# zhuangshaobin/Video-GPT

Hardware: AMD Instinct MI355X
Metric: denoised clip-tokens/sec (256^2, 8-frame next-clip, CFG, x1) (higher is better)
Workload: dtype bf16; 1 GPU; cfg-2 single-GPU inference: 256^2, C=4 cond + G=8 gen frames, CFG (B=2, L=3096, 5160 real tokens), Phi-3-mini-class denoiser 32 layers, x1 prediction, hipGraph sampler step; global_batch=1, parallelism=replicas x1, graph=True, condition_prefix_reuse=True, special_row_hoisting=True, attention_precision=bf16, full=False

## Files before the change

video-gpt_amd/csrc/glue.hip:

```cpp
#include "common.h"

namespace {

__global__ __launch_bounds__(256) void embed_gather_kernel(const int64_t* __restrict__ ids,
                                                           const bf16* __restrict__ table,
                                                           bf16* __restrict__ out, int64_t rows,
                                                           int H, int64_t vocab) {
    const int cpr = H >> 3;
    const int64_t total = rows * cpr;
    for (int64_t i = (int64_t)blockIdx.x * blockDim.x + threadIdx.x; i < total;
         i += (int64_t)gridDim.x * blockDim.x) {
        const int64_t row = i / cpr;
        const int c = (int)(i % cpr);
        int64_t id = ids[row];
        id = id < 0 ? 0 : (id >= vocab ? vocab - 1 : id);
        *reinterpret_cast<bf16x8*>(out + row * H + c * 8) =
            *reinterpret_cast<const bf16x8*>(table + id * H + c * 8);
    }
}

__global__ __launch_bounds__(256) void patch_embed_kernel(
    const bf16* __restrict__ x, const bf16* __restrict__ Wp, const bf16* __restrict__ bias,
    const bf16* __restrict__ pos, const int32_t* __restrict__ dst_row, bf16* __restrict__ seq,
    int C, int h, int w, int H, int pos_max) {
    __shared__ float patch[16][16];
    const int f = blockIdx.y;
    const int h2 = h >> 1, w2 = w >> 1;
    const int ntok = h2 * w2;
    const int t0 = blockIdx.x * 16;
    {
        const int tl = threadIdx.x >> 4, e = threadIdx.x & 15;
        const int t = t0 + tl;
        float v = 0.f;
        if (t < ntok) {
            const int ci = e >> 2, p = (e >> 1) & 1, q = e & 1;
            const int i = t / w2, j = t % w2;
            v = bf2f(x[(((int64_t)f * C + ci) * h + 2 * i + p) * w + 2 * j + q]);
        }
        patch[tl][e] = v;
    }
    __syncthreads();
    const int top = (pos_max - h2) / 2, left = (pos_max - w2) / 2;
    const int64_t row0 = dst_row[f];
    for (int c0 = threadIdx.x * 4; c0 < H; c0 += 256 * 4) {
        float wreg[4][16];
#pragma unroll
        for (int cc = 0; cc < 4; ++cc) {
            const bf16x8 lo = *reinterpret_cast<const bf16x8*>(Wp + (int64_t)(c0 + cc) * 16);
            const bf16x8 hi = *reinterpret_cast<const bf16x8*>(Wp + (int64_t)(c0 + cc) * 16 + 8);
#pragma unroll
            for (int e = 0; e < 8; ++e) {
                wreg[cc][e] = bf2f(lo[e]);
                wreg[cc][8 + e] = bf2f(hi[e]);
            }
        }
        const bf16x4 bv = *reinterpret_cast<const bf16x4*>(bias + c0);
        for (int tl = 0; tl < 16; ++tl) {
            const int t = t0 + tl;
            if (t >= ntok) break;
            const int i = t / w2, j = t % w2;
            const bf16x4 pv = *reinterpret_cast<const bf16x4*>(
                pos + ((int64_t)(top + i) * pos_max + left + j) * H + c0);
            bf16x4 o;
#pragma unroll
            for (int cc = 0; cc < 4; ++cc) {
                float acc = 0.f;
#pragma unroll
                for (int e = 0; e < 16; ++e) acc += wreg[cc][e] * patch[tl][e];
                o[cc] = f2bf(acc + bf2f(bv[cc]) + bf2f(pv[cc]));
            }
            *reinterpret_cast<bf16x4*>(seq + (row0 + t) * H + c0) = o;
        }
    }
}

__global__ void timestep_sinusoid_kernel(const float* __restrict__ t, const float* __restrict__ freqs,
                                         bf16* __restrict__ out, int n, int half) {
    const int idx = blockIdx.x * blockDim.x + threadIdx.x;
    if (idx >= n * half) return;
    const int m = idx / half, i = idx % half;
    const float arg = t[m] * freqs[i];
    out[(int64_t)m * 2 * half + i] = f2bf(cosf(arg));
    out[(int64_t)m * 2 * half + half + i] = f2bf(sinf(arg));
}

template <int MT>
__global__ __launch_bounds__(256) void linear_small_kernel(
    const bf16* __restrict__ x, const bf16* __restrict__ W, const bf16* __restrict__ bias,
    bf16* __restrict__ out, const int32_t* __restrict__ out_row, int M, int N, int K, int64_t ldx,
    int64_t ldo, int pre_act, int post_act) {
    const int lane = threadIdx.x & 63;
    const int wave = threadIdx.x >> 6;
    for (int n = blockIdx.x * 4 + wave; n < N; n += gridDim.x * 4) {
        float acc[MT];
#pragma unroll
        for (int m = 0; m < MT; ++m) acc[m] = 0.f;
        const bf16* wr = W + (int64_t)n * K;
        for (int k = lane * 8; k < K; k += 512) {
            const bf16x8 wv = *reinterpret_cast<const bf16x8*>(wr + k);
            float wf[8];
#pragma unroll
            for (int j = 0; j < 8; ++j) wf[j] = bf2f(wv[j]);
#pragma unroll
            for (int m = 0; m < MT; ++m) {
                if (m < M) {
                    const bf16x8 xv = *reinterpret_cast<const bf16x8*>(x + (int64_t)m * ldx + k);
#pragma unroll
                    for (int j = 0; j < 8; ++j) {
                        float xf = bf2f(xv[j]);
                        if (pre_act != VGPT_ACT_NONE) xf = bf2f(f2bf(act_apply(xf, pre_act)));
                        acc[m] += wf[j] * xf;
                    }
                }
            }
        }
        const float bn = bias ? bf2f(bias[n]) : 0.f;
#pragma unroll
        for (int m = 0; m < MT; ++m) {
            if (m < M) {
                float v = wave_sum(acc[m]) + bn;
                v = act_apply(v, post_act);
                if (lane == 0) {
                    const int64_t r = out_row ? (int64_t)out_row[m] : (int64_t)m;
                    out[r * ldo + n] = f2bf(v);
                }
            }
        }
    }
}

template <int NCH>
__global__ __launch_bounds__(256) void final_layer_kernel(
    const bf16* __restrict__ hidden, const int32_t* __restrict__ src_row, const bf16* __restrict__ mod,
    const bf16* __restrict__ Wf, const bf16* __restrict__ bfin, bf16* __restrict__ out, int C, int h,
    int w, int H, float eps) {
    const int lane = threadIdx.x & 63;
    const int wave = threadIdx.x >> 6;
    const int f = blockIdx.y;
    const int h2 = h >> 1, w2 = w >> 1;
    const int ntok = h2 * w2;
    const int t = blockIdx.x * 4 + wave;
    if (t >= ntok) return;
    const bf16* xr = hidden + ((int64_t)src_row[f] + t) * H;
    const bf16* shift = mod + (int64_t)f * 2 * H;
    const bf16* scale = shift + H;
    float v[NCH][8];
    float s1 = 0.f;
#pragma unroll
    for (int c = 0; c < NCH; ++c) {
        const int off = (c * 64 + lane) * 8;
        if (off < H) {
            const bf16x8 xv = *reinterpret_cast<const bf16x8*>(xr + off);
#pragma unroll
            for (int j = 0; j < 8; ++j) {
                v[c][j] = bf2f(xv[j]);
                s1 += v[c][j];
            }
        } else {
#pragma unroll
            for (int j = 0; j < 8; ++j) v[c][j] = 0.f;
        }
    }
    const float mean = wave_sum(s1) / (float)H;
    float s2 = 0.f;
#pragma unroll
    for (int c = 0; c < NCH; ++c) {
        const int off = (c * 64 + lane) * 8;
        if (off < H) {
#pragma unroll
            for (int j = 0; j < 8; ++j) {
                const float d = v[c][j] - mean;
                s2 += d * d;
            }
        }
    }
    const float rstd = rsqrtf(wave_sum(s2) / (float)H + eps);
#pragma unroll
    for (int c = 0; c < NCH; ++c) {
        const int off = (c * 64 + lane) * 8;
        if (off < H) {
            const bf16x8 sh = *reinterpret_cast<const bf16x8*>(shift + off);
            const bf16x8 sc = *reinterpret_cast<const bf16x8*>(scale + off);
#pragma unroll
            for (int j = 0; j < 8; ++j)
                v[c][j] = (v[c][j] - mean) * rstd * (1.0f + bf2f(sc[j])) + bf2f(sh[j]);
        }
    }
    float y = 0.f;
    for (int o = 0; o < 16; ++o) {
        float acc = 0.f;
#pragma unroll
        for (int c = 0; c < NCH; ++c) {
            const int off = (c * 64 + lane) * 8;
            if (off < H) {
                const bf16x8 wv = *reinterpret_cast<const bf16x8*>(Wf + (int64_t)o * H + off);
#pragma unroll
                for (int j = 0; j < 8; ++j) acc += v[c][j] * bf2f(wv[j]);
            }
        }
        acc = wave_sum(acc);
        if (lane == o) y = acc + bf2f(bfin[o]);
    }
    if (lane < 16) {
        const int c = lane % C, pq = lane / C;
        const int p = pq >> 1, q = pq & 1;
        const int i = t / w2, j = t % w2;
        out[(((int64_t)f * C + c) * h + 2 * i + p) * w + 2 * j + q] = f2bf(y);
    }
}

__global__ void set_timesteps_kernel(const float* sigma, const int32_t* step, float* ts, int n, int n_steps) {
    const int i = blockIdx.x * blockDim.x + threadIdx.x;
    const int st = *step;
    if (i < n && st >= 0 && st <= n_steps) ts[i] = sigma[st];
}

__global__ __launch_bounds__(256) void euler_cfg_kernel(float* __restrict__ z, bf16* __restrict__ zm,
                                                        const bf16* __restrict__ pred,
                                                        const float* __restrict__ sigma,
                                                        const int32_t* __restrict__ step, int n_steps, int n_frames,
                                                        int64_t elems, int pred_type, int use_cfg,
                                                        float cfg_scale) {
    const int st = *step;
    if (st < 0 || st >= n_steps) return;
    const float sg = sigma[st], sg_next = sigma[st + 1];
    const float dt = sg_next - sg;
    const float inv = 1.0f / (1.0f - sg);
    const int half = use_cfg ? n_frames / 2 : n_frames;
    const int64_t total = (int64_t)half * elems;
    for (int64_t i = (int64_t)blockIdx.x * blockDim.x + threadIdx.x; i < total;
         i += (int64_t)gridDim.x * blockDim.x) {
        float zc = z[i];
        float vc = bf2f(pred[i]);
        if (pred_type == VGPT_PRED_X1) vc = (vc - zc) * inv;
        if (use_cfg) {
            const int64_t iu = i + total;
            float zu = z[iu];
            float vu = bf2f(pred[iu]);
            if (pred_type == VGPT_PRED_X1) vu = (vu - zu) * inv;
            vc = vu + cfg_scale * (vc - vu);
            zu += dt * vc;
            z[iu] = zu;
            zm[iu] = f2bf(zu);
        }
        zc += dt * vc;
        z[i] = zc;
        zm[i] = f2bf(zc);
    }
}

__global__ void advance_kernel(int32_t* step) { *step += 1; }

__global__ __launch_bounds__(256) void cast_f32_bf16_kernel(const float* __restrict__ src,
                                                            bf16* __restrict__ dst, int64_t n) {
    for (int64_t i = (int64_t)blockIdx.x * blockDim.x + threadIdx.x; i < n;
         i += (int64_t)gridDim.x * blockDim.x)
        dst[i] = f2bf(src[i]);
}

}

VGPT_EXPORT int vgpt_embed_gather(const int64_t* ids, const void* table, void* out, int64_t rows,
                                  int64_t H, int64_t vocab, void* stream) {
    VGPT_REQUIRE(ids && table && out, VGPT_ERR_INVALID, "vgpt_embed_gather: null pointer");
    VGPT_REQUIRE(rows >= 0 && H > 0 && vocab > 0, VGPT_ERR_INVALID, "vgpt_embed_gather: bad shape");
    VGPT_REQUIRE(H % 8 == 0, VGPT_ERR_UNSUPPORTED, "vgpt_embed_gather: H must be a multiple of 8");
    if (rows == 0) return VGPT_OK;
    int grid = (int)std::min<int64_t>(cdiv(rows * (H / 8), 256), (int64_t)1 << 30);
    hipLaunchKernelGGL(embed_gather_kernel, dim3(grid), dim3(256), 0, (hipStream_t)stream, ids,
                       (const bf16*)table, (bf16*)out, rows, (int)H, vocab);
    VGPT_CHECK_LAUNCH("vgpt_embed_gather");
    return VGPT_OK;
}

VGPT_EXPORT int vgpt_patch_embed_fwd(const void* x, const void* Wp, const void* bias,
                                     const void* pos_embed, const int32_t* dst_row, void* seq,
                                     int n_frames, int C, int h, int w, int64_t H, int pos_max,
                                     void* stream) {
    VGPT_REQUIRE(x && Wp && bias && pos_embed && dst_row && seq, VGPT_ERR_INVALID,
                 "vgpt_patch_embed_fwd: null pointer");
    VGPT_REQUIRE(n_frames >= 0 && C > 0 && h > 0 && w > 0 && H > 0, VGPT_ERR_INVALID,
                 "vgpt_patch_embed_fwd: bad shape");
    VGPT_REQUIRE(C * 4 == 16 && h % 2 == 0 && w % 2 == 0, VGPT_ERR_UNSUPPORTED,
                 "vgpt_patch_embed_fwd: needs in_channels=4, patch 2, even latent size");
    VGPT_REQUIRE(H % 4 == 0, VGPT_ERR_UNSUPPORTED, "vgpt_patch_embed_fwd: H must be a multiple of 4");
    VGPT_REQUIRE(h / 2 <= pos_max && w / 2 <= pos_max, VGPT_ERR_INVALID,
                 "vgpt_patch_embed_fwd: latent larger than pos_embed_max_size");
    if (n_frames == 0) return VGPT_OK;
    const int ntok = (h / 2) * (w / 2);
    hipLaunchKernelGGL(patch_embed_kernel, dim3((unsigned)cdiv(ntok, 16), n_frames), dim3(256), 0,
                       (hipStream_t)stream, (const bf16*)x, (const bf16*)Wp, (const bf16*)bias,
                       (const bf16*)pos_embed, dst_row, (bf16*)seq, C, h, w, (int)H, pos_max);
    VGPT_CHECK_LAUNCH("vgpt_patch_embed_fwd");
    return VGPT_OK;
}

VGPT_EXPORT int vgpt_timestep_sinusoid(const float* t, const float* freqs, void* out, int n,
                                       int half, void* stream) {
    VGPT_REQUIRE(t && freqs && out, VGPT_ERR_INVALID, "vgpt_timestep_sinusoid: null pointer");
    VGPT_REQUIRE(n >= 0 && half > 0, VGPT_ERR_INVALID, "vgpt_timestep_sinusoid: bad shape");
    if (n == 0) return VGPT_OK;
    hipLaunchKernelGGL(timestep_sinusoid_kernel, dim3((unsigned)cdiv((int64_t)n * half, 256)),
                       dim3(256), 0, (hipStream_t)stream, t, freqs, (bf16*)out, n, half);
    VGPT_CHECK_LAUNCH("vgpt_timestep_sinusoid");
    return VGPT_OK;
}

VGPT_EXPORT int vgpt_linear_small(const void* x, const void* W, const void* bias, void* out,
                                  const int32_t* out_row, int M, int64_t N, int64_t K, int64_t ldx,
                                  int64_t ldo, int pre_act, int post_act, void* stream) {
    VGPT_REQUIRE(x && W && out, VGPT_ERR_INVALID, "vgpt_linear_small: null pointer");
    VGPT_REQUIRE(M >= 0 && N > 0 && K > 0, VGPT_ERR_INVALID, "vgpt_linear_small: bad shape");
    VGPT_REQUIRE(M <= 32, VGPT_ERR_UNSUPPORTED, "vgpt_linear_small: M=%d > 32", M);
    VGPT_REQUIRE(K % 8 == 0 && ldx % 8 == 0, VGPT_ERR_UNSUPPORTED,
                 "vgpt_linear_small: K and ldx must be multiples of 8");
    VGPT_REQUIRE(N < (1ll << 31) && K < (1ll << 31), VGPT_ERR_UNSUPPORTED,
                 "vgpt_linear_small: dimension too large");
    if (M == 0) return VGPT_OK;
    int grid = (int)std::min<int64_t>(cdiv(N, 4), 256 * 8);
    hipStream_t s = (hipStream_t)stream;
#define LS_CASE(MT)                                                                               \
    hipLaunchKernelGGL(linear_small_kernel<MT>, dim3(grid), dim3(256), 0, s, (const bf16*)x,       \
                       (const bf16*)W, (const bf16*)bias, (bf16*)out, out_row, M, (int)N, (int)K, \
                       ldx, ldo, pre_act, post_act)
    if (M <= 8) LS_CASE(8);
    else if (M <= 16) LS_CASE(16);
    else LS_CASE(32);
#undef LS_CASE
    VGPT_CHECK_LAUNCH("vgpt_linear_small");
    return VGPT_OK;
}

VGPT_EXPORT int vgpt_final_layer_fwd(const void* hidden, const int32_t* src_row, const void* mod,
                                     const void* Wf, const void* bf, void* out, int n_frames, int C,
                                     int h, int w, int64_t H, float eps, void* stream) {
    VGPT_REQUIRE(hidden && src_row && mod && Wf && bf && out, VGPT_ERR_INVALID,
                 "vgpt_final_layer_fwd: null pointer");
    VGPT_REQUIRE(n_frames >= 0 && C > 0 && h > 0 && w > 0 && H > 0, VGPT_ERR_INVALID,
                 "vgpt_final_layer_fwd: bad shape");
    VGPT_REQUIRE(C * 4 == 16 && h % 2 == 0 && w % 2 == 0, VGPT_ERR_UNSUPPORTED,
                 "vgpt_final_layer_fwd: needs out_channels=4, patch 2, even latent size");
    VGPT_REQUIRE(H % 8 == 0 && H <= 8 * 512, VGPT_ERR_UNSUPPORTED,
                 "vgpt_final_layer_fwd: H must be a multiple of 8 and <= 4096");
    if (n_frames == 0) return VGPT_OK;
    const int ntok = (h / 2) * (w / 2);
    dim3 grid((unsigned)cdiv(ntok, 4), n_frames);
    hipStream_t s = (hipStream_t)stream;
#define FL_CASE(N)                                                                              \
    case N:                                                                                     \
        hipLaunchKernelGGL(final_layer_kernel<N>, grid, dim3(256), 0, s, (const bf16*)hidden,   \
                           src_row, (const bf16*)mod, (const bf16*)Wf, (const bf16*)bf,         \
                           (bf16*)out, C, h, w, (int)H, eps);                                   \
        break;
    switch ((int)cdiv(H, 512)) {
        FL_CASE(1) FL_CASE(2) FL_CASE(3) FL_CASE(4) FL_CASE(5) FL_CASE(6) FL_CASE(7) FL_CASE(8)
    }
#undef FL_CASE
    VGPT_CHECK_LAUNCH("vgpt_final_layer_fwd");
    return VGPT_OK;
}

VGPT_EXPORT int vgpt_sampler_set_timesteps(const float* sigma, const int32_t* step, int n_steps, float* timesteps,
                                           int n, void* stream) {
    VGPT_REQUIRE(sigma && step && timesteps, VGPT_ERR_INVALID,
                 "vgpt_sampler_set_timesteps: null pointer");
    VGPT_REQUIRE(n >= 0 && n_steps > 0, VGPT_ERR_INVALID, "vgpt_sampler_set_timesteps: bad shape");
    if (n == 0) return VGPT_OK;
    hipLaunchKernelGGL(set_timesteps_kernel, dim3((unsigned)cdiv(n, 64)), dim3(64), 0,
                       (hipStream_t)stream, sigma, step, timesteps, n, n_steps);
    VGPT_CHECK_LAUNCH("vgpt_sampler_set_timesteps");
    return VGPT_OK;
}

VGPT_EXPORT int vgpt_euler_cfg_update(float* z, void* z_model, const void* pred, const float* sigma,
                                      const int32_t* step, int n_steps, int n_frames, int64_t elems, int pred_type,
                                      int use_cfg, float cfg_scale, void* stream) {
    VGPT_REQUIRE(z && z_model && pred && sigma && step, VGPT_ERR_INVALID,
                 "vgpt_euler_cfg_update: null pointer");
    VGPT_REQUIRE(n_frames >= 0 && elems >= 0 && n_steps > 0, VGPT_ERR_INVALID, "vgpt_euler_cfg_update: bad shape");
    VGPT_REQUIRE(pred_type == VGPT_PRED_V || pred_type == VGPT_PRED_X1, VGPT_ERR_INVALID,
                 "vgpt_euler_cfg_update: unknown prediction type %d", pred_type);
    VGPT_REQUIRE(!use_cfg || n_frames % 2 == 0, VGPT_ERR_INVALID,
                 "vgpt_euler_cfg_update: CFG needs an even number of frames");
    if (n_frames == 0 || elems == 0) return VGPT_OK;
    const int64_t total = (int64_t)(use_cfg ? n_frames / 2 : n_frames) * elems;
    int grid = (int)std::min<int64_t>(cdiv(total, 256), 2048);
    hipLaunchKernelGGL(euler_cfg_kernel, dim3(grid), dim3(256), 0, (hipStream_t)stream, z,
                       (bf16*)z_model, (const bf16*)pred, sigma, step, n_steps, n_frames, elems, pred_type,
                       use_cfg, cfg_scale);
    VGPT_CHECK_LAUNCH("vgpt_euler_cfg_update");
    return VGPT_OK;
}

__global__ __launch_bounds__(256) void copy_step_slab_kernel(const uint4* __restrict__ src, uint4* __restrict__ dst,
                                                             const int32_t* __restrict__ step, int n_steps, int64_t slab,
                                                             int64_t src_step_stride, int64_t src_layer_stride,
                                                             int64_t dst_layer_stride, int64_t total) {
    const int64_t i = (int64_t)blockIdx.x * 256 + threadIdx.x;
    if (i >= total) return;
    const int s = min(max(*step, 0), n_steps - 1);
    const int64_t l = i / slab, o = i % slab;
    dst[l * dst_layer_stride + o] = src[s * src_step_stride + l * src_layer_stride + o];
}

VGPT_EXPORT int vgpt_sampler_copy_step_rows(const void* src, void* dst, const int32_t* step, int n_steps, int n_layers,
                                            int64_t slab_bytes, int64_t src_step_stride_bytes,
                                            int64_t src_layer_stride_bytes, int64_t dst_layer_stride_bytes, void* stream) {
    VGPT_REQUIRE(src && dst && step, VGPT_ERR_INVALID, "vgpt_sampler_copy_step_rows: null pointer");
    VGPT_REQUIRE(n_steps > 0 && n_layers >= 0 && slab_bytes >= 0, VGPT_ERR_INVALID, "vgpt_sampler_copy_step_rows: bad shape");
    VGPT_REQUIRE(((slab_bytes | src_step_stride_bytes | src_layer_stride_bytes | dst_layer_stride_bytes) & 15) == 0 &&
                     (((uintptr_t)src | (uintptr_t)dst) & 15) == 0,
                 VGPT_ERR_UNSUPPORTED, "vgpt_sampler_copy_step_rows: sizes, strides and pointers must be multiples of 16 bytes");
    const int64_t slab = slab_bytes / 16, total = slab * n_layers;
    if (total == 0) return VGPT_OK;
    hipLaunchKernelGGL(copy_step_slab_kernel, dim3((unsigned)cdiv(total, 256)), dim3(256), 0, (hipStream_t)stream,
                       (const uint4*)src, (uint4*)dst, step, n_steps, slab, src_step_stride_bytes / 16,
                       src_layer_stride_bytes / 16, dst_layer_stride_bytes / 16, total);
    VGPT_CHECK_LAUNCH("vgpt_sampler_copy_step_rows");
    return VGPT_OK;
}

VGPT_EXPORT int vgpt_sampler_advance(int32_t* step, void* stream) {
    VGPT_REQUIRE(step, VGPT_ERR_INVALID, "vgpt_sampler_advance: null pointer");
    hipLaunchKernelGGL(advance_kernel, dim3(1), dim3(1), 0, (hipStream_t)stream, step);
    VGPT_CHECK_LAUNCH("vgpt_sampler_advance");
    return VGPT_OK;
}

VGPT_EXPORT int vgpt_cast_f32_to_bf16(const float* src, void* dst, int64_t n, void* stream) {
    VGPT_REQUIRE(src && dst, VGPT_ERR_INVALID, "vgpt_cast_f32_to_bf16: null pointer");
    VGPT_REQUIRE(n >= 0, VGPT_ERR_INVALID, "vgpt_cast_f32_to_bf16: bad shape");
    if (n == 0) return VGPT_OK;
    int grid = (int)std::min<int64_t>(cdiv(n, 256), 2048);
    hipLaunchKernelGGL(cast_f32_bf16_kernel, dim3(grid), dim3(256), 0, (hipStream_t)stream, src,
                       (bf16*)dst, n);
    VGPT_CHECK_LAUNCH("vgpt_cast_f32_to_bf16");
    return VGPT_OK;
}
```

Measured before the change: 73260 clip-tokens/s.

## Rework patch embed and small-M linear kernels for register and LDS reuse

Patch embedding now has each lane keep 8 output channels' weights in registers and loop over 8 tokens per wave. The grid is split over the hidden dim, with the old kernel kept as a fallback when H is not a multiple of 8. The small-M linear for M>8 now stages activation rows in LDS per K-chunk, and each wave computes 4 output columns at once, so x loads are reused across columns. These are small side kernels (embedding, timestep/adaLN projections) against a 32-layer transformer, so end-to-end impact is likely small, and the extra block barriers and register pressure may cost some occupancy.

Result: no change. 73300 clip-tokens/s, median of 2 (+0.0%).

```diff
diff --git a/video-gpt_amd/csrc/glue.hip b/video-gpt_amd/csrc/glue.hip
--- a/video-gpt_amd/csrc/glue.hip
+++ b/video-gpt_amd/csrc/glue.hip
@@ -19,7 +19,91 @@
     }
 }
 
+template <int N>
+__device__ __forceinline__ void wave_sum_n(float (&a)[N]) {
+#pragma unroll
+    for (int o = 32; o > 0; o >>= 1) {
+#pragma unroll
+        for (int i = 0; i < N; ++i) a[i] += __shfl_xor(a[i], o, 64);
+    }
+}
+
+constexpr int PE_TPW = 8, PE_TT = 4 * PE_TPW;
 __global__ __launch_bounds__(256) void patch_embed_kernel(
+    const bf16* __restrict__ x, const bf16* __restrict__ Wp, const bf16* __restrict__ bias,
+    const bf16* __restrict__ pos, const int32_t* __restrict__ dst_row, bf16* __restrict__ seq,
+    int C, int h, int w, int H, int pos_max) {
+#pragma clang fp contract(off)
+    __shared__ __attribute__((aligned(16))) float patch[PE_TT][16];
+    const int lane = threadIdx.x & 63;
+    const int wave = threadIdx.x >> 6;
+    const int f = blockIdx.y;
+    const int h2 = h >> 1, w2 = w >> 1;
+    const int ntok = h2 * w2;
+    const int t0 = blockIdx.x * PE_TT;
+    for (int idx = threadIdx.x; idx < PE_TT * 16; idx += 256) {
+        const int tl = idx >> 4, e = idx & 15;
+        const int t = t0 + tl;
+        float v = 0.f;
+        if (t < ntok) {
+            const int ci = e >> 2, p = (e >> 1) & 1, q = e & 1;
+            const int i = t / w2, j = t % w2;
+            v = bf2f(x[(((int64_t)f * C + ci) * h + 2 * i + p) * w + 2 * j + q]);
+        }
+        patch[tl][e] = v;
+    }
+    __syncthreads();
+    const int c0 = (blockIdx.z * 64 + lane) * 8;
+    if (c0 >= H) return;
+    const int top = (pos_max - h2) / 2, left = (pos_max - w2) / 2;
+    const int64_t row0 = dst_row[f];
+    float wreg[8][16];
+#pragma unroll
+    for (int cc = 0; cc < 8; ++cc) {
+        const bf16x8 lo = *reinterpret_cast<const bf16x8*>(Wp + (int64_t)(c0 + cc) * 16);
+        const bf16x8 hi = *reinterpret_cast<const bf16x8*>(Wp + (int64_t)(c0 + cc) * 16 + 8);
+#pragma unroll
+        for (int e = 0; e < 8; ++e) {
+            wreg[cc][e] = bf2f(lo[e]);
+            wreg[cc][8 + e] = bf2f(hi[e]);
+        }
+    }
+    const bf16x8 bv = *reinterpret_cast<const bf16x8*>(bias + c0);
+    bf16x8 pv[PE_TPW];
+#pragma unroll
+    for (int k = 0; k < PE_TPW; ++k) {
+        const int t = t0 + wave * PE_TPW + k;
+        if (t < ntok) {
+            const int i = t / w2, j = t % w2;
+            pv[k] = *reinterpret_cast<const bf16x8*>(pos + ((int64_t)(top + i) * pos_max + left + j) * H + c0);
+        }
+    }
+#pragma unroll
+    for (int k = 0; k < PE_TPW; ++k) {
+        const int tl = wave * PE_TPW + k;
+        const int t = t0 + tl;
+        if (t < ntok) {
+            float pt[16];
+#pragma unroll
+            for (int e4 = 0; e4 < 4; ++e4) {
+                const f32x4 p4 = *reinterpret_cast<const f32x4*>(&patch[tl][e4 * 4]);
+#pragma unroll
+                for (int e = 0; e < 4; ++e) pt[e4 * 4 + e] = p4[e];
+            }
+            bf16x8 o;
+#pragma unroll
+            for (int cc = 0; cc < 8; ++cc) {
+                float acc = wreg[cc][0] * pt[0];
+#pragma unroll
+                for (int e = 1; e < 16; ++e) acc = __builtin_fmaf(wreg[cc][e], pt[e], acc);
+                o[cc] = f2bf(acc + bf2f(bv[cc]) + bf2f(pv[k][cc]));
+            }
+            *reinterpret_cast<bf16x8*>(seq + (row0 + t) * H + c0) = o;
+        }
+    }
+}
+
+__global__ __launch_bounds__(256) void patch_embed4_kernel(
     const bf16* __restrict__ x, const bf16* __restrict__ Wp, const bf16* __restrict__ bias,
     const bf16* __restrict__ pos, const int32_t* __restrict__ dst_row, bf16* __restrict__ seq,
     int C, int h, int w, int H, int pos_max) {
@@ -123,6 +207,84 @@
                 if (lane == 0) {
                     const int64_t r = out_row ? (int64_t)out_row[m] : (int64_t)m;
                     out[r * ldo + n] = f2bf(v);
+                }
+            }
+        }
+    }
+}
+
+constexpr int LS_NC = 4;
+template <int MT>
+__global__ __launch_bounds__(256) void linear_small_lds_kernel(
+    const bf16* __restrict__ x, const bf16* __restrict__ W, const bf16* __restrict__ bias,
+    bf16* __restrict__ out, const int32_t* __restrict__ out_row, int M, int N, int K, int64_t ldx,
+    int64_t ldo, int pre_act, int post_act) {
+#pragma clang fp contract(off)
+    __shared__ __attribute__((aligned(16))) bf16 xs[MT][512];
+    const int lane = threadIdx.x & 63;
+    const int wave = threadIdx.x >> 6;
+    for (int64_t nb = (int64_t)blockIdx.x * (4 * LS_NC); nb < N; nb += (int64_t)gridDim.x * (4 * LS_NC)) {
+        const int64_t n0 = nb + wave * LS_NC;
+        float acc[MT][LS_NC];
+#pragma unroll
+        for (int m = 0; m < MT; ++m)
+#pragma unroll
+            for (int c = 0; c < LS_NC; ++c) acc[m][c] = 0.f;
+        for (int kc = 0; kc < K; kc += 512) {
+            __syncthreads();
+            for (int idx = threadIdx.x; idx < MT * 64; idx += 256) {
+                const int m = idx >> 6, k = kc + (idx & 63) * 8;
+                if (m < M && k < K) {
+                    bf16x8 xv = *reinterpret_cast<const bf16x8*>(x + (int64_t)m * ldx + k);
+                    if (pre_act != VGPT_ACT_NONE) {
+#pragma unroll
+                        for (int j = 0; j < 8; ++j) xv[j] = f2bf(act_apply(bf2f(xv[j]), pre_act));
+                    }
+                    *reinterpret_cast<bf16x8*>(&xs[m][(idx & 63) * 8]) = xv;
+                }
+            }
+            __syncthreads();
+            const int k = kc + lane * 8;
+            if (k < K) {
+                float wf[LS_NC][8];
+#pragma unroll
+                for (int c = 0; c < LS_NC; ++c) {
+                    if (n0 + c < N) {
+                        const bf16x8 wv = *reinterpret_cast<const bf16x8*>(W + (n0 + c) * K + k);
+#pragma unroll
+                        for (int j = 0; j < 8; ++j) wf[c][j] = bf2f(wv[j]);
+                    } else {
+#pragma unroll
+                        for (int j = 0; j < 8; ++j) wf[c][j] = 0.f;
+                    }
+                }
+#pragma unroll
+                for (int m = 0; m < MT; ++m) {
+                    if (m < M) {
+                        const bf16x8 xv = *reinterpret_cast<const bf16x8*>(&xs[m][lane * 8]);
+#pragma unroll
+                        for (int j = 0; j < 8; ++j) {
+                            const float xf = bf2f(xv[j]);
+#pragma unroll
+                            for (int c = 0; c < LS_NC; ++c) acc[m][c] = __builtin_fmaf(wf[c][j], xf, acc[m][c]);
+                        }
+                    }
+                }
+            }
+        }
+        float bn[LS_NC];
+#pragma unroll
+        for (int c = 0; c < LS_NC; ++c) bn[c] = (bias && n0 + c < N) ? bf2f(bias[n0 + c]) : 0.f;
+#pragma unroll
+        for (int m = 0; m < MT; ++m) {
+            if (m < M) {
+                wave_sum_n(acc[m]);
+                const int64_t r = out_row ? (int64_t)out_row[m] : (int64_t)m;
+#pragma unroll
+                for (int c = 0; c < LS_NC; ++c) {
+                    float v = acc[m][c] + bn[c];
+                    v = act_apply(v, post_act);
+                    if (lane == c && n0 + c < N) out[r * ldo + n0 + c] = f2bf(v);
                 }
             }
         }
@@ -288,9 +450,14 @@
                  "vgpt_patch_embed_fwd: latent larger than pos_embed_max_size");
     if (n_frames == 0) return VGPT_OK;
     const int ntok = (h / 2) * (w / 2);
-    hipLaunchKernelGGL(patch_embed_kernel, dim3((unsigned)cdiv(ntok, 16), n_frames), dim3(256), 0,
-                       (hipStream_t)stream, (const bf16*)x, (const bf16*)Wp, (const bf16*)bias,
-                       (const bf16*)pos_embed, dst_row, (bf16*)seq, C, h, w, (int)H, pos_max);
+    if (H % 8 == 0)
+        hipLaunchKernelGGL(patch_embed_kernel, dim3((unsigned)cdiv(ntok, PE_TT), n_frames, (unsigned)cdiv(H, 512)),
+                           dim3(256), 0, (hipStream_t)stream, (const bf16*)x, (const bf16*)Wp, (const bf16*)bias,
+                           (const bf16*)pos_embed, dst_row, (bf16*)seq, C, h, w, (int)H, pos_max);
+    else
+        hipLaunchKernelGGL(patch_embed4_kernel, dim3((unsigned)cdiv(ntok, 16), n_frames), dim3(256), 0,
+                           (hipStream_t)stream, (const bf16*)x, (const bf16*)Wp, (const bf16*)bias,
+                           (const bf16*)pos_embed, dst_row, (bf16*)seq, C, h, w, (int)H, pos_max);
     VGPT_CHECK_LAUNCH("vgpt_patch_embed_fwd");
     return VGPT_OK;
 }
@@ -317,15 +484,15 @@
     VGPT_REQUIRE(N < (1ll << 31) && K < (1ll << 31), VGPT_ERR_UNSUPPORTED,
                  "vgpt_linear_small: dimension too large");
     if (M == 0) return VGPT_OK;
-    int grid = (int)std::min<int64_t>(cdiv(N, 4), 256 * 8);
+    int grid = (int)std::min<int64_t>(cdiv(N, M <= 8 ? 4 : 4 * LS_NC), 256 * 8);
     hipStream_t s = (hipStream_t)stream;
-#define LS_CASE(MT)                                                                               \
-    hipLaunchKernelGGL(linear_small_kernel<MT>, dim3(grid), dim3(256), 0, s, (const bf16*)x,       \
-                       (const bf16*)W, (const bf16*)bias, (bf16*)out, out_row, M, (int)N, (int)K, \
-                       ldx, ldo, pre_act, post_act)
-    if (M <= 8) LS_CASE(8);
-    else if (M <= 16) LS_CASE(16);
-    else LS_CASE(32);
+#define LS_CASE(KERNEL)                                                                              \
+    hipLaunchKernelGGL(KERNEL, dim3(grid), dim3(256), 0, s, (const bf16*)x, (const bf16*)W,          \
+                       (const bf16*)bias, (bf16*)out, out_row, M, (int)N, (int)K, ldx, ldo, pre_act, \
+                       post_act)
+    if (M <= 8) LS_CASE(linear_small_kernel<8>);
+    else if (M <= 16) LS_CASE(linear_small_lds_kernel<16>);
+    else LS_CASE(linear_small_lds_kernel<32>);
 #undef LS_CASE
     VGPT_CHECK_LAUNCH("vgpt_linear_small");
     return VGPT_OK;
```
